# linjonathan/tropical_cyclone_risk

Measured on AMD Instinct MI355X. Metric: storm-steps/sec (100k-storm ensemble), higher is better.
Workload: dtype f64

## Files before the change

### include/tcrisk_hip.h

```cpp
#ifndef TCRISK_HIP_H
#define TCRISK_HIP_H

#include <stddef.h>
#include <stdint.h>

#ifdef __cplusplus
extern "C" {
#endif

#define TCR_ABI_VERSION 7
#define TCR_NW 4
#define TCR_NCOV 10
#define TCR_MAX_SERIES 32
#define TCR_N_BASINS 7

#define TCR_STATUS_GATED (-1)
#define TCR_STATUS_FINISHED 0
#define TCR_STATUS_EVENT 1
#define TCR_STATUS_STEP_FAIL (-2)
#define TCR_STATUS_STEP_OVERFLOW (-3)

#define TCR_FLAG_IS_TC 1
#define TCR_FLAG_ACCEPTED 2

// ... 49 lines not shown
    int32_t *nfev;
    int32_t *n_accept, *n_reject;
    int32_t *pad_state;
    int32_t tc_rows_only;
} tcr_tracks;

typedef struct {
    float *lon, *lat, *v, *m, *vmax;
    float *envw;
    int32_t *n_valid, *status, *flags, *nfev, *n_accept, *n_reject;
    int32_t *pad_state;
    int32_t tc_rows_only;
} tcr_tracks_f32;

int tcr_abi_version(void);
int tcr_ctx_create(int device, tcr_ctx **out);
int tcr_ctx_destroy(tcr_ctx *ctx);
const char *tcr_last_error(const tcr_ctx *ctx);

int tcr_params_set(tcr_ctx *ctx, const tcr_params *p);

int tcr_static_upload(tcr_ctx *ctx, const tcr_grid *hg, const double *land, const double *bathy);
int tcr_static_upload2(tcr_ctx *ctx, const tcr_grid *land_grid, const double *land,
                       const tcr_grid *bathy_grid, const double *bathy);
int tcr_static_store(tcr_ctx *ctx, int32_t pref);
int tcr_static_info(tcr_ctx *ctx, int32_t *mode, int64_t *bytes);
int tcr_fields_upload(tcr_ctx *ctx, int slot,
                      const tcr_grid *wg, const double *const mean[TCR_NW], const double *const cov[TCR_NCOV],
                      const tcr_grid *tg, const double *vpot, const double *chi,
                      const double *mld, const double *strat);
int tcr_rh_upload(tcr_ctx *ctx, int slot, const tcr_grid *rg, const double *rh_mid);
int tcr_slot_upload(tcr_ctx *ctx, int slot,
                    const tcr_grid *wg, const double *const mean[TCR_NW], const double *const cov[TCR_NCOV],
                    const tcr_grid *tg, const double *vpot, const double *chi, const double *mld, const double *strat,
                    const tcr_grid *rg, const double *rh_mid);
int tcr_stage_timing(tcr_ctx *ctx, double ms[5], int32_t reset);
int tcr_masks_upload(tcr_ctx *ctx, const tcr_grid *mg, const uint8_t *run_mask,
                     const uint8_t *const basin_masks[TCR_N_BASINS]);

int tcr_integrate_host(tcr_ctx *ctx, const tcr_storms *in, const tcr_tracks *out);
int tcr_integrate_dev(tcr_ctx *ctx, const tcr_storms *in_dev, const tcr_tracks *out_dev, void *stream);

int tcr_schedule_set(tcr_ctx *ctx, int32_t storms_per_lane);

typedef struct {
    int32_t waves;
    int32_t park;
    int32_t park_final;
    int32_t table_segments;
    int32_t prune;
    int32_t emit_grid_cap;
    int32_t copy_threads;
    int32_t table_factors;
} tcr_tune;
int tcr_tune_set(tcr_ctx *ctx, const tcr_tune *t);
int tcr_tune_get(tcr_ctx *ctx, tcr_tune *t);

int tcr_integrate_f32_dev(tcr_ctx *ctx, const tcr_storms *in_dev, const tcr_tracks_f32 *out_dev, void *stream);
int tcr_integrate_f32_host(tcr_ctx *ctx, const tcr_storms *in, const tcr_tracks_f32 *out);

typedef struct {
    int64_t n;
    double *lon0, *lat0, *v0, *m0, *h_bl;
    int32_t *slot;
    double *phases;
    int32_t *basin_idx;
    int32_t *seed_flags;
} tcr_seeds;
int tcr_seed_dev(tcr_ctx *ctx, uint64_t experiment_seed, int32_t year, int64_t cand0,
                 const tcr_seeds *out_dev, void *stream);
int tcr_seed_host(tcr_ctx *ctx, uint64_t experiment_seed, int32_t year, int64_t cand0,
                  const tcr_seeds *out_host);

int tcr_compact_dev(tcr_ctx *ctx, int64_t n, const int32_t *flags_dev, int32_t mask, int64_t max_out,
                    int32_t *idx_dev, int64_t *count_dev, void *stream);
int tcr_cell_order_dev(tcr_ctx *ctx, const tcr_seeds *cand_dev, int32_t *idx_dev, int64_t n, const int64_t *count_dev,
                       double cell_deg, void *stream);
int tcr_gather_seeds_dev(tcr_ctx *ctx, const tcr_seeds *src_dev, const int32_t *idx_dev, int64_t n_out,
                         const int64_t *count_dev, const tcr_seeds *dst_dev, uint64_t experiment_seed,
                         int32_t year, int64_t cand0, void *stream);
#define TCR_N_STATS 10
int tcr_stats_dev(tcr_ctx *ctx, int64_t n, const int64_t *n_dev, const tcr_tracks *tracks_dev, uint64_t *out_dev,
                  int32_t n_out, void *stream);
int tcr_pack_tracks_dev(tcr_ctx *ctx, const tcr_tracks *src_dev, const int32_t *idx_dev,
                        const int64_t *count_dev, int64_t cap, double *packed_dev, int64_t row_stride, void *stream);
int tcr_pack_tracks_f32_dev(tcr_ctx *ctx, const tcr_tracks_f32 *src_dev, const int32_t *idx_dev,
                            const int64_t *count_dev, int64_t cap, double *packed_dev, int64_t row_stride, void *stream);
int tcr_pack_tracks_meta_dev(tcr_ctx *ctx, const tcr_tracks *src_dev, int32_t f32, const int32_t *idx_dev,
                             const int64_t *count_dev, int64_t cap, double *packed_dev, int64_t row_stride,
                             const int32_t *cand_idx_dev, const int32_t *slot_dev, const int32_t *basin_idx_dev,
                             int64_t cand0, void *stream);
int tcr_seed_hist_dev(tcr_ctx *ctx, const tcr_seeds *cand_dev, int64_t cand0, const double *cutoff_dev,
                      int64_t *out_dev, void *stream);

typedef struct {
    int64_t n_cand;
    int64_t n_storms;
    tcr_seeds cand;
    tcr_seeds storms;
    int32_t *cand_idx;
    int64_t *n_passed;
    double cell_deg;
    int32_t exact_count;
    int32_t f32;
    tcr_tracks tracks;
    uint64_t *stats;
// ... 190 lines not shown
```

### tropical_cyclone_risk_amd/_lib.py

```python
import ctypes as C
import os

PKG_DIR = os.path.dirname(os.path.abspath(__file__))
LIB_PATH = os.path.join(PKG_DIR, 'libtcrisk_hip.so')

TCR_ABI_VERSION = 7
TCR_NW, TCR_NCOV, TCR_MAX_SERIES, TCR_N_BASINS = 4, 10, 32, 7
STATUS_GATED, STATUS_FINISHED, STATUS_EVENT, STATUS_STEP_FAIL, STATUS_STEP_OVERFLOW = -1, 0, 1, -2, -3
FLAG_IS_TC, FLAG_ACCEPTED = 1, 2
RAIN_TOTAL, RAIN_PEAK_RATE = 0, 1
SELECT_LDS_KEYS, SELECT_MAX_RANKS = 8192, 64
TAIL_MAX_K = 2048
STAGES = ('start', 'seed', 'select', 'order', 'gather', 'fourier', 'integrate', 'screen', 'select_tc', 'dense', 'emit', 'flags', 'stats', 'pack')
STATIC_MODES = ('f64', 'f64_split', 'pack16', 'u8_f32', 'pack64')
N_STATS = 10

DP = C.POINTER(C.c_double)
IP = C.POINTER(C.c_int32)
U8P = C.POINTER(C.c_uint8)

EXPORTS = ('tcr_abi_version', 'tcr_ctx_create', 'tcr_ctx_destroy', 'tcr_last_error',
           'tcr_params_set', 'tcr_static_upload', 'tcr_fields_upload', 'tcr_rh_upload', 'tcr_masks_upload',
           'tcr_integrate_host', 'tcr_integrate_dev', 'tcr_seed_dev', 'tcr_seed_host',
           'tcr_probe_rhs_host', 'tcr_fourier_table_host', 'tcr_timing_enable',
# ... 19 lines not shown
    _fields_ = [('nlon', C.c_int32), ('nlat', C.c_int32), ('lon', DP), ('lat', DP)]


class Params(C.Structure):
    _fields_ = [('Ck', C.c_double), ('epsilon', C.c_double), ('kappa', C.c_double),
                ('u_beta', C.c_double), ('v_beta', C.c_double), ('T_Fs', C.c_double),
                ('y_alpha', C.c_double * 2), ('m_alpha', C.c_double * 2),
                ('alpha_max', C.c_double * 2), ('alpha_min', C.c_double * 2),
                ('steering_coefs', C.c_double * 2),
                ('dt_out', C.c_double), ('total_time', C.c_double),
                ('rtol', C.c_double), ('atol', C.c_double), ('max_step', C.c_double),
                ('v_thresh', C.c_double), ('v_2d_thresh', C.c_double), ('vmax_thresh', C.c_double),
                ('v_dissipate', C.c_double), ('earth_R', C.c_double), ('box', C.c_double * 4),
                ('fs_amp', C.c_double), ('fs_wgt', C.c_double * TCR_MAX_SERIES),
                ('n_series', C.c_int32), ('n_steps', C.c_int32),
                ('coupled_track', C.c_int32), ('max_rk_steps', C.c_int32),
                ('seed_v_init', C.c_double), ('pi_gate', C.c_double), ('lat_vort_fac', C.c_double),
                ('lat_vort_power', C.c_double * TCR_N_BASINS),
                ('atm_bl_depth', C.c_double * TCR_N_BASINS),
                ('minit_a', C.c_double), ('minit_b', C.c_double),
                ('minit_c', C.c_double), ('minit_d', C.c_double)]


class Storms(C.Structure):
    _fields_ = [('n', C.c_int64), ('lon0', C.c_void_p), ('lat0', C.c_void_p), ('v0', C.c_void_p),
                ('m0', C.c_void_p), ('h_bl', C.c_void_p), ('slot', C.c_void_p), ('phases', C.c_void_p),
                ('n_dev', C.c_void_p)]


class Tracks(C.Structure):
    _fields_ = [('lon', C.c_void_p), ('lat', C.c_void_p), ('v', C.c_void_p), ('m', C.c_void_p),
                ('vmax', C.c_void_p), ('envw', C.c_void_p), ('n_valid', C.c_void_p),
                ('status', C.c_void_p), ('flags', C.c_void_p), ('nfev', C.c_void_p),
                ('n_accept', C.c_void_p), ('n_reject', C.c_void_p), ('pad_state', C.c_void_p),
                ('tc_rows_only', C.c_int32)]


class Seeds(C.Structure):
    _fields_ = [('n', C.c_int64), ('lon0', C.c_void_p), ('lat0', C.c_void_p), ('v0', C.c_void_p),
                ('m0', C.c_void_p), ('h_bl', C.c_void_p), ('slot', C.c_void_p),
                ('phases', C.c_void_p), ('basin_idx', C.c_void_p), ('seed_flags', C.c_void_p)]


class Round(C.Structure):
    _fields_ = [('n_cand', C.c_int64), ('n_storms', C.c_int64), ('cand', Seeds), ('storms', Seeds),
                ('cand_idx', C.c_void_p), ('n_passed', C.c_void_p), ('cell_deg', C.c_double),
                ('exact_count', C.c_int32), ('f32', C.c_int32), ('tracks', Tracks),
                ('stats', C.c_void_p), ('acc_idx', C.c_void_p), ('n_accepted', C.c_void_p),
                ('packed', C.c_void_p), ('pack_cap', C.c_int64), ('pack_stride', C.c_int64), ('seed_hist', C.c_void_p),
                ('n_expected', C.c_int64)]


class Tune(C.Structure):
    _fields_ = [(k, C.c_int32) for k in ('waves', 'park', 'park_final', 'table_segments', 'prune', 'emit_grid_cap', 'copy_threads', 'table_factors')]


class HazardTracks(C.Structure):
    _fields_ = [('n_trk', C.c_int64), ('n_t', C.c_int64), ('row_stride', C.c_int64), ('lon', C.c_void_p), ('lat', C.c_void_p),
                ('vmax', C.c_void_p), ('n_group', C.c_int32), ('group_off', C.POINTER(C.c_int64))]


class LandGrid(C.Structure):
    _fields_ = [('nlon', C.c_int64), ('nlat', C.c_int64), ('lon', C.c_void_p), ('lat', C.c_void_p), ('land', C.c_void_p)]


class ClimGrid(C.Structure):
    _fields_ = [('lon0', C.c_double), ('dlon', C.c_double), ('lat0', C.c_double), ('dlat', C.c_double), ('nlon', C.c_int64),
                ('nlat', C.c_int64)]


class ClimOut(C.Structure):
    _fields_ = [(k, C.c_void_p) for k in ('track', 'exceed', 'genesis', 'lmi', 'pdi', 'genesis_k', 'lmi_v', 'lmi_k', 'pdi_storm')]


class WindTracks(C.Structure):
    _fields_ = [('n_trk', C.c_int64), ('n_t', C.c_int64), ('row_stride', C.c_int64)] + \
        [(k, C.c_void_p) for k in ('lon', 'lat', 'v', 'u250', 'v250', 'u850', 'v850', 'rmax_km')] + \
        [('n_group', C.c_int32), ('group_off', C.POINTER(C.c_int64))]


class WindParams(C.Structure):
    _fields_ = [('dt_s', C.c_double), ('ck_cd', C.c_double), ('r_out_km', C.c_double), ('rmax_const_km', C.c_double),
                ('substeps', C.c_int32)]


class LossParams(C.Structure):
    _fields_ = [('v_thresh', C.c_double), ('v_half', C.c_double)]


class RainParams(C.Structure):
    _fields_ = [('dt_s', C.c_double), ('r_out_km', C.c_double), ('v_lo_kt', C.c_double), ('v_hi_kt', C.c_double),
                ('a', C.c_double * 4), ('b', C.c_double * 4), ('substeps', C.c_int32), ('stat', C.c_int32)]


class TcrError(RuntimeError):
    pass


_lib = None


def _pin_hip_runtime():
    import importlib.util
    import sys
    if 'torch' in sys.modules:
        return
    try:
# ... 145 lines not shown
```

### tropical_cyclone_risk_amd/csrc/tcr_abi.hip

```cpp
#include <hip/hip_runtime.h>

#include <cstdlib>

#include "tcr_kernels.hip"
#include "tcr_seed.hip"
#include "tcr_compact.hip"
#include "tcr_prep.hip"
#include "tcr_thermo.hip"
#ifdef TCR_EXPERIMENTS
#include "tcr_experiments.h"
#endif

#include "tcr_host.h"
#include "tcr_ctx.h"
#include "tcr_stage.hip"
#include "tcr_integrate.hip"
#include "tcr_preprocess.hip"
#include "tcr_round.hip"

namespace {

long env_long(const char *name, long dflt)
{
    const char *e = getenv(name);
    return e ? atol(e) : dflt;
}
tcr_tune tune_from_env()
{
    tcr_tune t;
    t.waves = (int32_t)env_long("TCR_WAVES", -1);
    t.park = (int32_t)std::min<long>(env_long("TCR_PARK", -1), 63);
    t.park_final = (int32_t)env_long("TCR_PARK_FINAL", -1);
    t.table_segments = (int32_t)env_long("TCR_TABLE_SEGMENTS", -1);
    t.prune = (int32_t)env_long("TCR_PRUNE", -1);
    t.emit_grid_cap = (int32_t)env_long("TCR_EMIT_GRID_CAP", -1);
    t.copy_threads = (int32_t)env_long("TCR_COPY_THREADS", -1);
    t.table_factors = (int32_t)env_long("TCR_TABLE_FACTORS", -1);
    return t;
}

}

extern "C" {

int tcr_abi_version(void) { return TCR_ABI_VERSION; }

const char *tcr_last_error(const tcr_ctx *ctx) { return ctx ? ctx->err.c_str() : g_create_error.c_str(); }

int tcr_ctx_create(int device, tcr_ctx **out)
{
    if (!out) return fail(nullptr, "tcr_ctx_create: out is NULL");
    *out = nullptr;
    int count = 0;
    hipError_t e = hipGetDeviceCount(&count);
    if (e != hipSuccess || count <= 0)
        return fail(nullptr, "no HIP device available (%s); this library has no CPU fallback",
                    e != hipSuccess ? hipGetErrorString(e) : "device count is 0");
    if (device < 0 || device >= count) return fail(nullptr, "tcr_ctx_create: device index out of range");
    tcr_ctx *ctx = new tcr_ctx();
    ctx->device = device;
    ctx->tune = tune_from_env();
    if (hipSetDevice(device) != hipSuccess || hipStreamCreate(&ctx->stream) != hipSuccess) {
        delete ctx;
        return fail(nullptr, "tcr_ctx_create: hipSetDevice/hipStreamCreate failed");
    }
    hipDeviceProp_t prop;
    if (hipGetDeviceProperties(&prop, device) == hipSuccess && prop.multiProcessorCount > 0) {
        ctx->cu_count = prop.multiProcessorCount;
        if (prop.sharedMemPerBlock < kCellScanLds) {
            delete ctx;
            return fail(nullptr, "tcr_ctx_create: this library is built for gfx950 (160 KB of LDS per CU); the device offers less than k_cell_scan's 67 KB per workgroup");
        }
    }
    if (ctx->ws.d_queue.alloc_bytes(kQueueWords * sizeof(unsigned long long)) != hipSuccess ||
        ctx->ws.d_tc_count.alloc_bytes(64) != hipSuccess || ctx->rd.d_round_key.alloc_bytes(64) != hipSuccess) {
        delete ctx;
        return fail(nullptr, "tcr_ctx_create: hipMalloc failed");
    }
    *out = ctx;
    return 0;
}

int tcr_ctx_destroy(tcr_ctx *ctx)
{
    if (!ctx) return 0;
    (void)hipSetDevice(ctx->device);
    (void)hipStreamSynchronize(ctx->stream);
    delete ctx;
    return 0;
}
// ... 71 lines not shown
```

### tropical_cyclone_risk_amd/csrc/tcr_integrate.hip

```cpp
#pragma once
#include <cmath>

#include "tcr_stage.hip"

namespace {

unsigned integrate_waves(const tcr_ctx *ctx, int64_t n, int wps)
{
    (void)wps;
    const int64_t simds = (int64_t)ctx->cu_count * 4;
    int64_t waves = (n + kWave - 1) / kWave;
    if (ctx->tune.waves > 0) return (unsigned)(ctx->tune.waves < waves ? ctx->tune.waves : waves);
    if (waves > simds) waves = (n >= simds * kWave * 4) ? 2 * simds : simds;
    else if (ctx->storms_per_lane > 1) {
        const int64_t w = (n + (int64_t)kWave * ctx->storms_per_lane - 1) / ((int64_t)kWave * ctx->storms_per_lane);
        waves = std::max<int64_t>(std::min<int64_t>(waves, 16), w);
    }
    return (unsigned)(waves < 1 ? 1 : waves);
}

int park_threshold(const tcr_ctx *ctx, unsigned waves, int wps)
{
    if (ctx->tune.park >= 0) return ctx->tune.park > 63 ? 63 : ctx->tune.park;
    (void)wps;
// ... 120 lines not shown
            int list_stride = 1;
            if (part == kFsRest) {
                list = reinterpret_cast<const int64_t *>(park) + 13;
                list_stride = kParkRec;
            } else if (!fused) {
                if (W.d_pf.grow(ctx, (size_t)tiles * kFsMfmaKSteps * 32) < 0) return -1;
                hipLaunchKernelGGL(k_phase_factors_frag, dim3((unsigned)std::min<int64_t>(tiles, 8192)), dim3(256), 0, st, P, n, n_dev, phases,
                                   reinterpret_cast<double *>(W.d_pf.p), nullptr, nullptr, z);
            }
            const double *p = fused ? phases : reinterpret_cast<const double *>(W.d_pf.p);
            const int groups = part == kFsAll ? kFsMfmaColGroups : 1;
            int64_t want = (int64_t)ctx->cu_count * kFsMfmaWgsPerCu * (4 / kFsMfmaWaves) / groups;
#ifdef TCR_EXPERIMENTS
            want = tcr_exp::fs_workgroups(want, groups);
#endif
            const unsigned wgs = (unsigned)std::min<int64_t>(tiles, std::max<int64_t>(1, want));
            const dim3 grid(wgs, groups), block(64 * kFsMfmaWaves);
            const BatchReset none{};
            with_flags(part == kFsRest, fused, [&](auto REST, auto FUSED) {
                constexpr bool rest = decltype(REST)::value, fu = decltype(FUSED)::value;
                hipLaunchKernelGGL((k_fourier_mfma<R, rest, fu>), grid, block, 0, st, P, n, n_dev, W.fs_period, W.d_sc_table.p, p, fs,
                                   rest ? 1 : 0, list, list_stride, park_count, (fu && !rest) ? z : none);
            });
        } else {
            hipLaunchKernelGGL(k_phase_factors, dim3((unsigned)((nf + 255) / 256)), dim3(256), 0, st, P, n, n_dev, phases, W.d_pf.p);
            hipLaunchKernelGGL(k_fourier_periodic<R>, dim3((unsigned)n), dim3(kFsThreads), lds, st, P, n, n_dev,
                               W.fs_period, W.d_sc_table.p, W.d_pf.p, fs);
        }
    } else {
        const int64_t total = n * (int64_t)P.n_steps;
        hipLaunchKernelGGL(k_fourier_direct<R>, dim3((unsigned)((total + 255) / 256)), dim3(256), 0, st, P, n, n_dev, phases, fs);
    }
    HIPCHK(ctx, hipGetLastError());
    return 0;
}

template <typename R>
int integrate_impl(tcr_ctx *ctx, const tcr_storms *in, const TracksT<R> out, void *stream_, uint64_t *stats = nullptr,
                   const int64_t *stats_n_dev = nullptr, int64_t n_expected = 0)
{
    hipStream_t st = enter(ctx, stream_);
    if (!st) return -1;
    IntegrateWs &W = ctx->ws;
    const int64_t n = in->n;
    if (n < 0) return fail(ctx, "tcr_integrate: negative n");
    if (n == 0) return 0;
    const tcr_params &P = ctx->prm;
    const size_t ns = (size_t)P.n_steps;
    constexpr size_t REC = (size_t)step_rec_doubles<R>();
    if (W.d_fs.grow(ctx, ((size_t)n * ns * 4 * sizeof(R) + 7) / 8) < 0) return -1;
    const int max_rk = P.max_rk_steps > 0 ? P.max_rk_steps : 64;
    if (W.d_srec.grow(ctx, (size_t)n * max_rk * REC) < 0) return -1;
    if (max_rk > 65535) return fail(ctx, "tcr_params.max_rk_steps must be <= 65535");
    if (W.d_sidx.grow(ctx, ((size_t)n * ns * sizeof(uint16_t) + 7) / 8 * 4) < 0) return -1;
    R *fs = reinterpret_cast<R *>(W.d_fs.p);
    EvalKT<R> EK{};
    bool affine = false;
    if (eval_k_ready<R>(ctx, EK, &affine, st)) return -1;

    hipEvent_t *ev = nullptr;
    if (ctx->tr.timing && !ctx->capturing && timing_events(ctx, &ev)) return -1;
    if (ev) HIPCHK(ctx, hipEventRecord(ev[0], st));
    const int wps = std::is_same<R, double>::value ? TCR_INT_WPS : TCR_INT_WPS_F32;
    unsigned waves = integrate_waves(ctx, (n_expected > 0 && n_expected < n) ? n_expected : n, wps);
    const int thr = park_threshold(ctx, waves, wps);
    const unsigned final_waves = park_final_waves(ctx);
    const bool segmented = kFsMfmaColGroups == 2 && thr > 0 && waves > final_waves && kMaxPasses > 1 && fourier_on_matrix_cores(ctx) &&
                           (int)P.n_steps > kFsSegSamples + 16 && ctx->tune.table_segments != 0;
    int prune_sample = -1;
    if (out.tc_rows_only && ctx->tune.prune != 0) {
        const double t2d = 2 * 86400.0, step_out = P.total_time / (double)(P.n_steps - 1);
        const int j = (int)floor(t2d / step_out);
        if (j >= 1 && j < P.n_steps - 1 && ts_host(P, j) == t2d) prune_sample = j;
    }
    const bool in_flight = prune_sample >= 0;
    if (!in_flight && W.d_vrec.grow(ctx, (size_t)n * max_rk * kVRec) < 0) return -1;
    if (out.tc_rows_only && W.d_tc_idx.grow(ctx, (size_t)n) < 0) return -1;
    unsigned long long *tc_count = reinterpret_cast<unsigned long long *>(W.d_tc_count.p);
    {
        BatchReset z{};
        z.queue = W.d_queue.p; z.queue_words = (int)kQueueWords;
        if (in_flight) { z.flags = out.flags; z.n_flags = n; }
        if (out.tc_rows_only) z.tc_count = tc_count;
        if (launch_fourier<R>(ctx, n, in->n_dev, in->phases, fs, st, segmented ? kFsFirst : kFsAll, nullptr, nullptr, &z)) return -1;
    }
    STAGE(TCR_STAGE_FOURIER);
    if (ev) HIPCHK(ctx, hipEventRecord(ev[1], st));
    {
        KArgsT<R> a{};
        a.P = P; a.D = dev_fields(ctx); a.K = EK; a.n = n; a.n_dev = in->n_dev;
        a.lon0 = in->lon0; a.lat0 = in->lat0; a.v0 = in->v0; a.m0 = in->m0; a.h_bl = in->h_bl;
        a.slot = in->slot; a.phases = in->phases; a.fs = fs; a.srec = W.d_srec.p; a.vrec = in_flight ? nullptr : W.d_vrec.p; a.max_rk_steps = max_rk;
        a.n_valid = out.n_valid; a.status = out.status; a.nfev = out.nfev;
        a.n_accept = out.n_accept; a.n_reject = out.n_reject;
        a.queue = W.d_queue.p;
        a.prune_sample = prune_sample;
        if (in_flight) {
            a.tc_list = W.d_tc_idx.p; a.tc_count = tc_count;
        }
        const size_t park_items = segmented ? (size_t)n : (size_t)waves * kWave;
        if (thr > 0 && W.d_park[0].grow(ctx, park_items * kParkRec) < 0) return -1;
        if (thr > 0 && W.d_park[1].grow(ctx, park_items * kParkRec) < 0) return -1;
        const bool probe = std::is_same<R, double>::value && W.d_probe;
        if (probe) { a.probe = W.d_probe; a.probe_cap = W.probe_cap; }
        bool seg_events = false;
        for (int pass = 0; pass < kMaxPasses; ++pass) {
            const bool last = thr <= 0 || waves <= final_waves || pass == kMaxPasses - 1;
            a.pass = pass;
            a.fill_pct = pass_fill_pct();
            a.threshold = last ? 0 : thr;
            a.park_in = W.d_park[(pass + 1) & 1].p;
            a.park_out = W.d_park[pass & 1].p;
            a.t_limit = (segmented && pass == 0) ? ts_host(P, kFsSegSamples - 2) : 1e300;
            launch_integrate(a, affine, probe, ctx->sg.static_mode, waves, st);
            if (last) break;
            if (segmented && pass == 0) {
                if (ev) HIPCHK(ctx, hipEventRecord(ev[4], st));
                if (launch_fourier<R>(ctx, n, in->n_dev, in->phases, fs, st, kFsRest, W.d_park[0].p, W.d_queue.p + kMaxPasses)) return -1;
                if (ev) HIPCHK(ctx, hipEventRecord(ev[5], st));
                seg_events = true;
                continue;
            }
            waves = (unsigned)(((size_t)waves * (size_t)(thr - 1) + kWave - 1) / kWave);
        }
        if (ev && !seg_events) { HIPCHK(ctx, hipEventRecord(ev[4], st)); HIPCHK(ctx, hipEventRecord(ev[5], st)); }
    }
    STAGE(TCR_STAGE_INTEGRATE);
    if (W.d_steps) HIPCHK(ctx, hipMemcpyAsync(W.d_steps, W.d_srec.p, sizeof(double) * (size_t)n * max_rk * REC, hipMemcpyDeviceToDevice, st));
    if (ev) HIPCHK(ctx, hipEventRecord(ev[2], st));
    {
        EArgsT<R> a{};
        a.P = P; a.D = dev_fields(ctx); a.n = n; a.n_dev = in->n_dev; a.max_rk_steps = max_rk; a.srec = W.d_srec.p; a.vrec = in_flight ? nullptr : W.d_vrec.p; a.fs = fs;
        a.slot = in->slot; a.n_valid = out.n_valid; a.status = out.status; a.n_accept = out.n_accept;
        a.lon = out.lon; a.lat = out.lat; a.v = out.v; a.m = out.m; a.vmax = out.vmax;
        a.envw = out.envw; a.flags = out.flags; a.pad_state = out.pad_state;
        a.K = EK;
        const unsigned chunks = (unsigned)((ns + kPostThreads - 1) / kPostThreads);
        if (out.tc_rows_only) {
            if (!in_flight) {
                a.tc_list = W.d_tc_idx.p; a.tc_count = tc_count;
                hipLaunchKernelGGL(k_screen<R>, dim3((unsigned)((n + kScreenStorms - 1) / kScreenStorms)), dim3(kScreenThreads), 0, st, a);
            }
            STAGE(TCR_STAGE_SCREEN);
            STAGE(TCR_STAGE_SELECT_TC);
            a.list = W.d_tc_idx.p; a.count = W.d_tc_count.p;
        }
        int64_t cap = kEmitGridCap;
        if (ctx->tune.emit_grid_cap > 0) cap = ctx->tune.emit_grid_cap;
        const unsigned gx = (out.tc_rows_only && n > 2 * cap) ? (unsigned)cap : (unsigned)n;
        hipLaunchKernelGGL(k_dense<R>, dim3(gx), dim3(kWave), 0, st, a, W.d_sidx.p);
        STAGE(TCR_STAGE_DENSE);
        const unsigned ex = gx;
        auto emit = [&](unsigned rows, bool overflow) {
            with_flags(affine, overflow, [&](auto A, auto OV) {
                hipLaunchKernelGGL((k_emit<R, decltype(A)::value, decltype(OV)::value>), dim3(rows, chunks), dim3(kPostThreads), 0, st, a, W.d_sidx.p);
            });
        };
        emit(ex, false);
        if ((int64_t)ex < n) {
            a.item_base = ex;
            emit((unsigned)std::min<int64_t>(n - ex, 256), true);
            a.item_base = 0;
        }
        STAGE(TCR_STAGE_EMIT);
        hipLaunchKernelGGL(k_flags<R>, dim3((unsigned)((n + 255) / 256)), dim3(256), 0, st, P, n, out.n_valid,
                           out.status, out.v, out.flags, out.pad_state, out.tc_rows_only ? 1 : 0, a.n_dev, out.nfev,
                           reinterpret_cast<unsigned long long *>(stats), stats_n_dev);
        STAGE(TCR_STAGE_FLAGS);
    }
    if (ev) HIPCHK(ctx, hipEventRecord(ev[3], st));
    HIPCHK(ctx, hipGetLastError());
    return 0;
}

int storms_upload(tcr_ctx *ctx, DevBuf &B, const tcr_storms *in, tcr_storms *d, const char *who, bool need_m0 = true)
{
    const size_t n = (size_t)in->n;
    for (size_t i = 0; i < n; ++i)
        if (!slot_staged(ctx, in->slot[i])) return fail(ctx, "%s: storm references a slot that is not staged", who);
    *d = tcr_storms{};
    d->n = in->n;
    d->lon0 = B.put(in->lon0, n); d->lat0 = B.put(in->lat0, n); d->v0 = B.put(in->v0, n);
    d->m0 = (need_m0 || in->m0) ? B.put(in->m0, n) : nullptr;
    d->h_bl = B.put(in->h_bl, n); d->slot = B.put(in->slot, n);
    d->phases = B.put(in->phases, n * 4 * (size_t)ctx->prm.n_series);
    d->n_dev = nullptr;
    if (!d->lon0 || !d->lat0 || !d->v0 || ((need_m0 || in->m0) && !d->m0) || !d->h_bl || !d->slot || !d->phases)
        return fail(ctx, "%s: device allocation / upload failed", who);
    return 0;
}

template <typename R, typename T>
int integrate_host_impl(tcr_ctx *ctx, const tcr_storms *in, const T *out)
{
    if (ready(ctx, false)) return -1;
    if (!in || !out) return fail(ctx, "tcr_integrate_host: NULL argument");
    if (!enter(ctx)) return -1;
    const size_t n = (size_t)in->n, ns = (size_t)ctx->prm.n_steps;
    if (n == 0) return 0;
    DevBuf B;
    tcr_storms di{};
    if (storms_upload(ctx, B, in, &di, "tcr_integrate_host")) return -1;
    TracksT<R> dout{};
    dout.lon = B.get<R>(n * ns); dout.lat = B.get<R>(n * ns); dout.v = B.get<R>(n * ns);
    dout.m = B.get<R>(n * ns); dout.vmax = B.get<R>(n * ns); dout.envw = B.get<R>(n * ns * 4);
    dout.n_valid = B.get<int32_t>(n); dout.status = B.get<int32_t>(n); dout.flags = B.get<int32_t>(n);
    dout.nfev = B.get<int32_t>(n); dout.n_accept = B.get<int32_t>(n); dout.n_reject = B.get<int32_t>(n);
    if (!dout.lon || !dout.lat || !dout.v || !dout.m || !dout.vmax || !dout.envw || !dout.n_valid || !dout.status ||
// ... 302 lines not shown
```

### tropical_cyclone_risk_amd/csrc/tcr_kernels.hip

```cpp
#include "tcr_device.h"

namespace tcr {

template <typename R>
struct KArgsT {
    tcr_params P;
    DevFields D;
    EvalKT<R> K;
    int64_t n;
    const int64_t *n_dev;
    const double *lon0, *lat0, *v0, *m0, *h_bl;
    const int32_t *slot;
    const double *phases;
    R *fs;
    double *srec;
    int32_t *n_valid, *status, *nfev, *n_accept, *n_reject;
    unsigned long long *queue;
    int max_rk_steps;
    int pass;
    int threshold;
    int fill_pct;
    const double *park_in;
    double *park_out;
    double t_limit;
// ... 794 lines not shown
};
using EArgs = EArgsT<double>;
static_assert(sizeof(EvalKT<double>) % 8 == 0 && sizeof(EvalKT<float>) % 8 == 0, "EvalK is copied to LDS in eight-byte words");
constexpr int kBitAny15 = 1 << 8, kBitVmax = 1 << 9;
constexpr int kBitListed = 1 << 10;
#ifndef TCR_POST_THREADS
#define TCR_POST_THREADS 128
#endif
constexpr int kPostThreads = TCR_POST_THREADS;
#ifndef TCR_EMIT_GRID_CAP
#define TCR_EMIT_GRID_CAP 8192
#endif
constexpr int64_t kEmitGridCap = TCR_EMIT_GRID_CAP;
constexpr int kEmitSlotCache = 32;
#ifndef TCR_EMIT_WPS
#define TCR_EMIT_WPS 3
#endif
#ifndef TCR_SHADOW_WPS
#define TCR_SHADOW_WPS 6
#endif

template <typename R>
__device__ __forceinline__ const R *rec_body(const double *rec) { return reinterpret_cast<const R *>(rec + kStepHdr); }

template <typename R>
__global__ __launch_bounds__(kWave) void k_dense(EArgsT<R> a, uint16_t *__restrict__ sidx)
{
    const tcr_params &P = a.P;
    const int64_t n_items = a.list ? *a.count : a.n;
    const int64_t n_exist = a.list ? n_items : n_eff(a.n, a.n_dev);
    for (int64_t item = blockIdx.x; item < n_items; item += gridDim.x) {
        if (item >= n_exist) {
            if (threadIdx.x == 0) a.flags[item] = 0;
            continue;
        }
        const int64_t sid = a.list ? (int64_t)a.list[item] : item;
        const int ns = P.n_steps;
        const int n = a.n_valid[sid];
        int nst = a.n_accept[sid];
        nst = nst < a.max_rk_steps ? nst : a.max_rk_steps;
        if (threadIdx.x == 0) a.flags[sid] = a.list ? kBitListed : 0;
        constexpr int REC = step_rec_doubles<R>();
        typedef typename VecT<R, 4>::type V4;
        const int c = threadIdx.x & 3;
        for (int j0 = 0; j0 < nst; j0 += kWave / 4) {
            const int j = j0 + (threadIdx.x >> 2);
            const bool on = j < nst;
            double *rj = const_cast<double *>(a.srec) + (sid * (int64_t)a.max_rk_steps + (on ? j : 0)) * REC;
            R *body = reinterpret_cast<R *>(rj + kStepHdr);
            R kq[7];
            for (int q = 0; q < 7; ++q) kq[q] = body[4 + q * 4 + c];
            const double t_old = rj[0], t_new = rj[2];
            R Q[4];
            for (int k = 0; k < 4; ++k) {
                R acc = R(0.0);
                for (int q = 0; q < 7; ++q) acc += kq[q] * R(RK_P[q][k]);
                Q[k] = acc;
            }
            if (on) {
                V4 qv; qv[0] = Q[0]; qv[1] = Q[1]; qv[2] = Q[2]; qv[3] = Q[3];
                *reinterpret_cast<V4 *>(body + 4 + c * 4) = qv;
                if (c == 0) {
                    const int i_lo = (j == 0) ? 0 : samples_upto(P, t_old);
                    int i_hi = samples_upto(P, t_new);
                    i_hi = i_hi < n ? i_hi : n;
                    for (int i = i_lo; i < i_hi; ++i) sidx[(size_t)sid * ns + i] = (uint16_t)j;
                }
            }
        }
    }
}

template <typename R>
__device__ __forceinline__ R haversine_same_lat_km(const tcr_params &P, R lon1, R lon2, R lat)
{
    const R d = R(kPi / 180.0);
    lon1 *= d; lon2 *= d; lat *= d;
    const R sb = sin((lon2 - lon1) / R(2)), c = cos(lat);
    const R aa = R(0.0) + c * c * (sb * sb);
    return R(P.earth_R / 1000.) * (R(2) * asin(sqrt(aa)));
}

template <typename R>
__device__ __forceinline__ R haversine_same_lon_km(const tcr_params &P, R lat1, R lat2)
{
    const R d = R(kPi / 180.0);
    lat1 *= d; lat2 *= d;
    const R sa = sin((lat2 - lat1) / R(2));
    const R aa = sa * sa;
    return R(P.earth_R / 1000.) * (R(2) * asin(sqrt(aa)));
}

template <typename R>
__device__ __forceinline__ R vmax_at(const tcr_params &P, R lon, R lat, R v, R us, R vs, R lom, R lam, R lop, R lap)
{
    const R dlon = R(0.5) * (sign_of(lop - lom) * haversine_same_lat_km<R>(P, lop, lom, lat));
    const R dlat = R(0.5) * (sign_of(lap - lam) * haversine_same_lon_km<R>(P, lap, lam));
    const R ut = dlon * R(1000.) / (R)P.dt_out, vt = dlat * R(1000.) / (R)P.dt_out;
    const R G = fmin(R(1.), R(0.8) + R(0.35) * (R(1.) + tanh((lat - R(35.)) / R(10.))));
    const R Ui = G * ut + R(0.1) * us * v / R(15.);
    const R Vi = G * vt + R(0.1) * vs * v / R(15.);
    const R mag = sqrt(Ui * Ui + Vi * Vi);
    const R fac = np_min((v * R(0.50)) / mag, R(1.0));
    const R msin = (mag == R(0.0)) ? R(0.0) : Ui / mag;
    const R mcos = (mag == R(0.0)) ? R(1.0) : Vi / mag;
    const R ug = v * msin + Ui * fac;
    const R vg = v * mcos + Vi * fac;
    return sqrt(ug * ug + vg * vg);
}

template <typename R, int NC>
__device__ __forceinline__ void dense_at(const double *__restrict__ srec_storm, int step, double te, R (&ye)[NC])
{
    typedef typename VecT<R, 4>::type V4;
    const double *rec = srec_storm + (size_t)step * step_rec_doubles<R>();
    const double2 h0 = *reinterpret_cast<const double2 *>(rec);
    const V4 *body = reinterpret_cast<const V4 *>(rec + kStepHdr);
    const R hh = (R)h0.y;
    const R x = (R)((te - h0.x) / h0.y);
    const R p1 = x, p2 = p1 * x, p3 = p2 * x, p4 = p3 * x;
    const V4 y0 = body[0];
#pragma unroll
    for (int c = 0; c < NC; ++c) {
        const V4 q = body[1 + c];
        R acc = R(0.0);
        acc += q[0] * p1; acc += q[1] * p2; acc += q[2] * p3; acc += q[3] * p4;
        ye[c] = hh * acc + y0[c];
    }
}

template <typename R, bool AFFINE, bool LIST>
__global__ __launch_bounds__(kPostThreads, TCR_SHADOW_WPS) void k_emit(EArgsT<R> a, const uint16_t *__restrict__ sidx)
{
    __shared__ EvalKT<R> K_lds;
    __shared__ const R *s_wind[kEmitSlotCache];
    const tcr_params &P = a.P;
    const int64_t n_items = a.list ? *a.count : n_eff(a.n, a.n_dev);
    if ((int64_t)blockIdx.x + (LIST ? a.item_base : 0) >= n_items) return;
    const int ns = P.n_steps;
    const int i = blockIdx.y * kPostThreads + threadIdx.x;
    const R nan = (R)__longlong_as_double(0x7ff8000000000000LL);
    for (unsigned w = threadIdx.x; w < sizeof(EvalKT<R>) / 8; w += kPostThreads)
        reinterpret_cast<uint64_t *>(&K_lds)[w] = reinterpret_cast<const uint64_t *>(&a.K)[w];
    if (threadIdx.x < kEmitSlotCache && (int)threadIdx.x < a.D.n_slots) s_wind[threadIdx.x] = slot_wind<R>(a.D.slots[threadIdx.x]);
    __syncthreads();
    int64_t item = blockIdx.x + (LIST ? a.item_base : 0);
#pragma unroll 1
    do {
        int koff = 0;
        asm volatile("" : "+s"(koff));
        const EvalKT<R> &K = *reinterpret_cast<const EvalKT<R> *>(reinterpret_cast<const char *>(&K_lds) + koff);
        const int64_t sid = a.list ? (int64_t)a.list[item] : item;
        const int n = a.n_valid[sid];
        const int slot_id = a.slot[sid];
        const uint16_t *sidx_storm = sidx + (size_t)sid * ns;
        const int my_step = (i < ns) ? sidx_storm[i] : 0;
        const size_t o = (size_t)sid * ns + i;
        typedef typename VecT<R, 4>::type V4;
        const bool valid = i < n;
        const double *srec_storm = a.srec + sid * (int64_t)a.max_rk_steps * step_rec_doubles<R>();
        R ye[4] = {0, 0, 0, 0}, w[4] = {0, 0, 0, 0};
        if (valid) {
            const double te = ts_at(P, i);
            dense_at<R, 4>(srec_storm, my_step, te, ye);
            const R *wind = (slot_id < kEmitSlotCache) ? s_wind[slot_id] : slot_wind<R>(a.D.slots[slot_id]);
            env_winds<R, AFFINE>(K, wind, a.fs + sid * ns * 4, ye[0], ye[1], te, w);
            a.lon[o] = ye[0]; a.lat[o] = ye[1]; a.v[o] = ye[2]; a.m[o] = ye[3];
            V4 wv; wv[0] = w[0]; wv[1] = w[1]; wv[2] = w[2]; wv[3] = w[3];
            *reinterpret_cast<V4 *>(a.envw + o * 4) = wv;
        }
        const int lane = threadIdx.x & 63;
        R lom = __shfl_up(ye[0], 1), lam = __shfl_up(ye[1], 1);
        R lop = __shfl_down(ye[0], 1), lap = __shfl_down(ye[1], 1);
        if (valid && n > 1) {
            if (lane == 0 && i > 0) {
                R q[2];
                dense_at<R, 2>(srec_storm, sidx_storm[i - 1], ts_at(P, i - 1), q);
                lom = q[0]; lam = q[1];
            }
            if (lane == 63 && i < n - 1) {
                R q[2];
                dense_at<R, 2>(srec_storm, sidx_storm[i + 1], ts_at(P, i + 1), q);
                lop = q[0]; lap = q[1];
            }
            const R lop_in = lop, lap_in = lap, lom_in = lom, lam_in = lam;
            if (i == 0) { lom = R(2) * ye[0] - lop_in; lam = R(2) * ye[1] - lap_in; }
            if (i == n - 1) { lop = R(2) * ye[0] - lom_in; lap = R(2) * ye[1] - lam_in; }
            const R vm = vmax_at<R>(P, ye[0], ye[1], ye[2], w[0] - w[2], w[1] - w[3], lom, lam, lop, lap);
            a.vmax[o] = vm;
            const bool hit_v = ye[2] >= (R)P.v_thresh, hit_vm = vm >= (R)P.vmax_thresh;
            const int bits = (__ballot(hit_v) ? kBitAny15 : 0) | (__ballot(hit_vm) ? kBitVmax : 0);
            if (bits && lane == (__ffsll((long long)__ballot(true)) - 1)) atomicOr(a.flags + sid, bits);
        } else if (valid) {
            a.vmax[o] = nan;
            if (ye[2] >= (R)P.v_thresh) atomicOr(a.flags + sid, kBitAny15);
        } else {
            int pad_to = a.pad_state ? a.pad_state[sid] : ns;
            pad_to = (pad_to < 0 || pad_to > ns) ? ns : pad_to;
            if (i < pad_to) {
                a.lon[o] = nan; a.lat[o] = nan; a.v[o] = nan; a.m[o] = nan; a.vmax[o] = nan;
                V4 nv; nv[0] = nan; nv[1] = nan; nv[2] = nan; nv[3] = nan;
                *reinterpret_cast<V4 *>(a.envw + o * 4) = nv;
            }
        }
    } while (LIST && (item += gridDim.x) < n_items);
}

constexpr int kScreenThreads = 256;
constexpr int kScreenGroup = 16;
constexpr int kScreenStorms = kScreenThreads / kScreenGroup;

template <typename R>
__global__ __launch_bounds__(kScreenThreads, TCR_SHADOW_WPS) void k_screen(EArgsT<R> a)
{
    __shared__ R cap[kScreenStorms][3];
    const tcr_params &P = a.P;
    const int g = threadIdx.x / kScreenGroup, l = threadIdx.x % kScreenGroup;
    const int64_t sid = (int64_t)blockIdx.x * kScreenStorms + g;
    const bool on = sid < a.n;
    const bool exists = sid < n_eff(a.n, a.n_dev);
    const int ns = P.n_steps;
    int n = 0, nst = 0, st = TCR_STATUS_GATED;
    if (exists) {
        n = a.n_valid[sid]; nst = a.n_accept[sid]; st = a.status[sid];
        nst = nst < a.max_rk_steps ? nst : a.max_rk_steps;
    }
    const double step_out = P.total_time / (double)(ns - 1);
    const double t2d = 2 * 86400.0;
    const bool clamp2d = n > 0 && t2d >= ts_at(P, n - 1);
    const int j2d = clamp2d ? n - 1 : (int)floor(t2d / step_out);
    bool any15 = false;
    const double *vrec_storm = a.vrec + sid * (int64_t)a.max_rk_steps * kVRec;
    typedef StepVT<R> StepV;
    auto load_step = [&](int j) {
        const double2 *rj = reinterpret_cast<const double2 *>(vrec_storm + (size_t)j * kVRec);
        const double2 r0 = rj[0], r1 = rj[1], r2 = rj[2], r3 = rj[3], r4 = rj[4], r5 = rj[5];
        StepV s;
        s.t_old = r0.x; s.h64 = r0.y;
        const double t_new = r1.x;
        s.hh = (R)s.h64; s.y0 = (R)r1.y;
        const R kq[7] = {(R)r2.x, (R)r2.y, (R)r3.x, (R)r3.y, (R)r4.x, (R)r4.y, (R)r5.x};
        dense_v_row<R>(kq, s.Q);
        s.i_lo = (j == 0) ? 0 : samples_upto(P, s.t_old);
        s.i_hi = samples_upto(P, t_new);
        s.i_hi = s.i_hi < n ? s.i_hi : n;
        return s;
    };
    auto v_at = [&](const StepV &s, int i) -> R { return dense_v_at<R>(P, s, i); };
    auto caps = [&](const StepV &s) {
        if (s.i_lo <= j2d && j2d < s.i_hi) cap[g][0] = v_at(s, j2d);
        if (s.i_lo <= j2d + 1 && j2d + 1 < s.i_hi) cap[g][1] = v_at(s, j2d + 1);
        if (s.i_lo <= n - 1 && n - 1 < s.i_hi) cap[g][2] = v_at(s, n - 1);
    };
    const bool has0 = l < nst && n > 0;
    StepV s0{};
    if (has0) { s0 = load_step(l); caps(s0); }
    for (int j = l + kScreenGroup; j < nst && n > 0; j += kScreenGroup) caps(load_step(j));
    __syncthreads();
// ... 240 lines not shown
```

Measured before the change: 11.25 billion.

## Fold dense-output step conversion into emit kernel, dropping the separate dense pass

Makes fusion the default: the emit kernel now builds the sample-to-step ownership map in LDS, computes the dense-output polynomial coefficients for the RK steps covering its chunk, and evaluates the track samples and edge neighbours from shared memory. This removes the separate k_dense launch and the global sidx buffer along with its write and read traffic. The old two-pass path stays available through a TCR_DENSE_PASS tune knob. The cost is more shared memory, extra block syncs per group of steps, and recomputing coefficients for steps shared by neighbouring chunks.

Result: no change. 11.33 billion, median of 6 (+0.7%).

```diff
diff --git a/include/tcrisk_hip.h b/include/tcrisk_hip.h
--- a/include/tcrisk_hip.h
+++ b/include/tcrisk_hip.h
@@ -125,6 +125,7 @@
     int32_t emit_grid_cap;
     int32_t copy_threads;
     int32_t table_factors;
+    int32_t dense_pass;
 } tcr_tune;
 int tcr_tune_set(tcr_ctx *ctx, const tcr_tune *t);
 int tcr_tune_get(tcr_ctx *ctx, tcr_tune *t);
diff --git a/tropical_cyclone_risk_amd/_lib.py b/tropical_cyclone_risk_amd/_lib.py
--- a/tropical_cyclone_risk_amd/_lib.py
+++ b/tropical_cyclone_risk_amd/_lib.py
@@ -95,7 +95,7 @@
 
 
 class Tune(C.Structure):
-    _fields_ = [(k, C.c_int32) for k in ('waves', 'park', 'park_final', 'table_segments', 'prune', 'emit_grid_cap', 'copy_threads', 'table_factors')]
+    _fields_ = [(k, C.c_int32) for k in ('waves', 'park', 'park_final', 'table_segments', 'prune', 'emit_grid_cap', 'copy_threads', 'table_factors', 'dense_pass')]
 
 
 class HazardTracks(C.Structure):
diff --git a/tropical_cyclone_risk_amd/csrc/tcr_abi.hip b/tropical_cyclone_risk_amd/csrc/tcr_abi.hip
--- a/tropical_cyclone_risk_amd/csrc/tcr_abi.hip
+++ b/tropical_cyclone_risk_amd/csrc/tcr_abi.hip
@@ -36,6 +36,7 @@
     t.emit_grid_cap = (int32_t)env_long("TCR_EMIT_GRID_CAP", -1);
     t.copy_threads = (int32_t)env_long("TCR_COPY_THREADS", -1);
     t.table_factors = (int32_t)env_long("TCR_TABLE_FACTORS", -1);
+    t.dense_pass = (int32_t)env_long("TCR_DENSE_PASS", -1);
     return t;
 }
 
diff --git a/tropical_cyclone_risk_amd/csrc/tcr_integrate.hip b/tropical_cyclone_risk_amd/csrc/tcr_integrate.hip
--- a/tropical_cyclone_risk_amd/csrc/tcr_integrate.hip
+++ b/tropical_cyclone_risk_amd/csrc/tcr_integrate.hip
@@ -196,7 +196,8 @@
     const int max_rk = P.max_rk_steps > 0 ? P.max_rk_steps : 64;
     if (W.d_srec.grow(ctx, (size_t)n * max_rk * REC) < 0) return -1;
     if (max_rk > 65535) return fail(ctx, "tcr_params.max_rk_steps must be <= 65535");
-    if (W.d_sidx.grow(ctx, ((size_t)n * ns * sizeof(uint16_t) + 7) / 8 * 4) < 0) return -1;
+    const bool fold = ctx->tune.dense_pass <= 0;
+    if (!fold && W.d_sidx.grow(ctx, ((size_t)n * ns * sizeof(uint16_t) + 7) / 8 * 4) < 0) return -1;
     R *fs = reinterpret_cast<R *>(W.d_fs.p);
     EvalKT<R> EK{};
     bool affine = false;
@@ -224,7 +225,7 @@
     {
         BatchReset z{};
         z.queue = W.d_queue.p; z.queue_words = (int)kQueueWords;
-        if (in_flight) { z.flags = out.flags; z.n_flags = n; }
+        if (in_flight || fold) { z.flags = out.flags; z.n_flags = n; }
         if (out.tc_rows_only) z.tc_count = tc_count;
         if (launch_fourier<R>(ctx, n, in->n_dev, in->phases, fs, st, segmented ? kFsFirst : kFsAll, nullptr, nullptr, &z)) return -1;
     }
@@ -292,12 +293,14 @@
         int64_t cap = kEmitGridCap;
         if (ctx->tune.emit_grid_cap > 0) cap = ctx->tune.emit_grid_cap;
         const unsigned gx = (out.tc_rows_only && n > 2 * cap) ? (unsigned)cap : (unsigned)n;
-        hipLaunchKernelGGL(k_dense<R>, dim3(gx), dim3(kWave), 0, st, a, W.d_sidx.p);
+        if (!fold) hipLaunchKernelGGL(k_dense<R>, dim3(gx), dim3(kWave), 0, st, a, W.d_sidx.p);
         STAGE(TCR_STAGE_DENSE);
         const unsigned ex = gx;
         auto emit = [&](unsigned rows, bool overflow) {
             with_flags(affine, overflow, [&](auto A, auto OV) {
-                hipLaunchKernelGGL((k_emit<R, decltype(A)::value, decltype(OV)::value>), dim3(rows, chunks), dim3(kPostThreads), 0, st, a, W.d_sidx.p);
+                constexpr bool AF = decltype(A)::value, ov = decltype(OV)::value;
+                if (fold) hipLaunchKernelGGL((k_emit<R, AF, ov>), dim3(rows, chunks), dim3(kPostThreads), 0, st, a);
+                else hipLaunchKernelGGL((k_emit_sidx<R, AF, ov>), dim3(rows, chunks), dim3(kPostThreads), 0, st, a, W.d_sidx.p);
             });
         };
         emit(ex, false);
diff --git a/tropical_cyclone_risk_amd/csrc/tcr_kernels.hip b/tropical_cyclone_risk_amd/csrc/tcr_kernels.hip
--- a/tropical_cyclone_risk_amd/csrc/tcr_kernels.hip
+++ b/tropical_cyclone_risk_amd/csrc/tcr_kernels.hip
@@ -870,11 +870,7 @@
             for (int q = 0; q < 7; ++q) kq[q] = body[4 + q * 4 + c];
             const double t_old = rj[0], t_new = rj[2];
             R Q[4];
-            for (int k = 0; k < 4; ++k) {
-                R acc = R(0.0);
-                for (int q = 0; q < 7; ++q) acc += kq[q] * R(RK_P[q][k]);
-                Q[k] = acc;
-            }
+            dense_v_row<R>(kq, Q);
             if (on) {
                 V4 qv; qv[0] = Q[0]; qv[1] = Q[1]; qv[2] = Q[2]; qv[3] = Q[3];
                 *reinterpret_cast<V4 *>(body + 4 + c * 4) = qv;
@@ -947,11 +943,38 @@
     }
 }
 
-template <typename R, bool AFFINE, bool LIST>
-__global__ __launch_bounds__(kPostThreads, TCR_SHADOW_WPS) void k_emit(EArgsT<R> a, const uint16_t *__restrict__ sidx)
+template <typename R, int NC>
+__device__ __forceinline__ void dense_at(const double2 h0, const R *__restrict__ body_lds, double te, R (&ye)[NC])
+{
+    typedef typename VecT<R, 4>::type V4;
+    const V4 *body = reinterpret_cast<const V4 *>(body_lds);
+    const R hh = (R)h0.y;
+    const R x = (R)((te - h0.x) / h0.y);
+    const R p1 = x, p2 = p1 * x, p3 = p2 * x, p4 = p3 * x;
+    const V4 y0 = body[0];
+#pragma unroll
+    for (int c = 0; c < NC; ++c) {
+        const V4 q = body[1 + c];
+        R acc = R(0.0);
+        acc += q[0] * p1; acc += q[1] * p2; acc += q[2] * p3; acc += q[3] * p4;
+        ye[c] = hh * acc + y0[c];
+    }
+}
+
+constexpr int kFoldSteps = 16;
+constexpr int kFoldBody = 20;
+static_assert(kFoldSteps * 4 <= kPostThreads, "k_emit's fold: a lane per (step, component)");
+
+template <typename R, bool AFFINE, bool LIST, bool FOLD>
+__device__ __forceinline__ void emit_body(const EArgsT<R> &a, const uint16_t *__restrict__ sidx)
 {
     __shared__ EvalKT<R> K_lds;
     __shared__ const R *s_wind[kEmitSlotCache];
+    __shared__ double2 s_hdr[FOLD ? kFoldSteps : 1];
+    __shared__ __attribute__((aligned(32))) R s_body[FOLD ? kFoldSteps * kFoldBody : 4];
+    __shared__ uint16_t s_own[FOLD ? kPostThreads + 2 : 2];
+    __shared__ R s_v[FOLD ? kPostThreads : 1];
+    __shared__ R s_edge[kPostThreads / 64][4];
     const tcr_params &P = a.P;
     const int64_t n_items = a.list ? *a.count : n_eff(a.n, a.n_dev);
     if ((int64_t)blockIdx.x + (LIST ? a.item_base : 0) >= n_items) return;
@@ -971,34 +994,97 @@
         const int64_t sid = a.list ? (int64_t)a.list[item] : item;
         const int n = a.n_valid[sid];
         const int slot_id = a.slot[sid];
-        const uint16_t *sidx_storm = sidx + (size_t)sid * ns;
-        const int my_step = (i < ns) ? sidx_storm[i] : 0;
+        const uint16_t *sidx_storm = FOLD ? nullptr : sidx + (size_t)sid * ns;
+        const int my_step = (!FOLD && i < ns) ? sidx_storm[i] : 0;
         const size_t o = (size_t)sid * ns + i;
         typedef typename VecT<R, 4>::type V4;
         const bool valid = i < n;
         const double *srec_storm = a.srec + sid * (int64_t)a.max_rk_steps * step_rec_doubles<R>();
         R ye[4] = {0, 0, 0, 0}, w[4] = {0, 0, 0, 0};
+        const bool edge_m = valid && n > 1 && (threadIdx.x & 63) == 0 && i > 0, edge_p = valid && n > 1 && (threadIdx.x & 63) == 63 && i < n - 1;
+        if (FOLD) {
+            if (a.list && blockIdx.y == 0 && threadIdx.x == 0) atomicOr(a.flags + sid, kBitListed);
+            const int i0 = blockIdx.y * kPostThreads;
+            if (i0 < n) {
+                constexpr int REC = step_rec_doubles<R>();
+                int nst = a.n_accept[sid];
+                nst = nst < a.max_rk_steps ? nst : a.max_rk_steps;
+                const int w_lo = i0 > 0 ? i0 - 1 : 0, w_hi = (i0 + kPostThreads + 1 < n) ? i0 + kPostThreads + 1 : n;
+                for (int j = threadIdx.x; j < nst; j += kPostThreads) {
+                    const double *rj = srec_storm + (size_t)j * REC;
+                    const double t_old = rj[0], t_new = rj[2];
+                    int i_lo = (j == 0) ? 0 : samples_upto(P, t_old);
+                    int i_hi = samples_upto(P, t_new);
+                    i_hi = i_hi < w_hi ? i_hi : w_hi;
+                    i_lo = i_lo > w_lo ? i_lo : w_lo;
+                    for (int k = i_lo; k < i_hi; ++k) s_own[k - (i0 - 1)] = (uint16_t)j;
+                }
+                __syncthreads();
+                const int j_top = nst > 0 ? nst - 1 : 0;
+                auto own = [&](int k) { const int j = s_own[k - (i0 - 1)]; return j < j_top ? j : j_top; };
+                const int j_first = own(w_lo), j_last = own(w_hi - 1);
+                const int my_j = valid ? own(i) : 0, jm = edge_m ? own(i - 1) : 0, jp = edge_p ? own(i + 1) : 0;
+                const double te = ts_at(P, i);
+#pragma unroll 1
+                for (int jb = j_first; jb <= j_last; jb += kFoldSteps) {
+                    if (jb != j_first) __syncthreads();
+                    const int s = threadIdx.x >> 2, c = threadIdx.x & 3, j = jb + s;
+                    if (s < kFoldSteps && j <= j_last) {
+                        const double *rj = srec_storm + (size_t)j * REC;
+                        const R *body = rec_body<R>(rj);
+                        R kq[7];
+                        for (int q = 0; q < 7; ++q) kq[q] = body[4 + q * 4 + c];
+                        const R y_old = body[c];
+                        if (c == 0) s_hdr[s] = *reinterpret_cast<const double2 *>(rj);
+                        R Q[4];
+                        dense_v_row<R>(kq, Q);
+                        V4 qv; qv[0] = Q[0]; qv[1] = Q[1]; qv[2] = Q[2]; qv[3] = Q[3];
+                        *reinterpret_cast<V4 *>(&s_body[s * kFoldBody + 4 + c * 4]) = qv;
+                        s_body[s * kFoldBody + c] = y_old;
+                    }
+                    __syncthreads();
+                    const unsigned span = (unsigned)(j_last - jb < kFoldSteps - 1 ? j_last - jb : kFoldSteps - 1);
+                    if (valid && (unsigned)(my_j - jb) <= span) dense_at<R, 4>(s_hdr[my_j - jb], &s_body[(my_j - jb) * kFoldBody], te, ye);
+                    if (edge_m && (unsigned)(jm - jb) <= span) {
+                        R q[2];
+                        dense_at<R, 2>(s_hdr[jm - jb], &s_body[(jm - jb) * kFoldBody], ts_at(P, i - 1), q);
+                        s_edge[threadIdx.x >> 6][0] = q[0]; s_edge[threadIdx.x >> 6][1] = q[1];
+                    }
+                    if (edge_p && (unsigned)(jp - jb) <= span) {
+                        R q[2];
+                        dense_at<R, 2>(s_hdr[jp - jb], &s_body[(jp - jb) * kFoldBody], ts_at(P, i + 1), q);
+                        s_edge[threadIdx.x >> 6][2] = q[0]; s_edge[threadIdx.x >> 6][3] = q[1];
+                    }
+                }
+            }
+        }
         if (valid) {
             const double te = ts_at(P, i);
-            dense_at<R, 4>(srec_storm, my_step, te, ye);
+            if (!FOLD) dense_at<R, 4>(srec_storm, my_step, te, ye);
+            if (FOLD) { a.m[o] = ye[3]; s_v[threadIdx.x] = ye[2]; asm volatile("" ::: "memory"); }
             const R *wind = (slot_id < kEmitSlotCache) ? s_wind[slot_id] : slot_wind<R>(a.D.slots[slot_id]);
             env_winds<R, AFFINE>(K, wind, a.fs + sid * ns * 4, ye[0], ye[1], te, w);
-            a.lon[o] = ye[0]; a.lat[o] = ye[1]; a.v[o] = ye[2]; a.m[o] = ye[3];
+            if (FOLD) { asm volatile("" ::: "memory"); ye[2] = s_v[threadIdx.x]; }
+            a.lon[o] = ye[0]; a.lat[o] = ye[1]; a.v[o] = ye[2];
+            if (!FOLD) a.m[o] = ye[3];
             V4 wv; wv[0] = w[0]; wv[1] = w[1]; wv[2] = w[2]; wv[3] = w[3];
             *reinterpret_cast<V4 *>(a.envw + o * 4) = wv;
         }
-        const int lane = threadIdx.x & 63;
+        const int lane = FOLD ? (int)__builtin_amdgcn_mbcnt_hi(~0u, __builtin_amdgcn_mbcnt_lo(~0u, 0u)) : (int)(threadIdx.x & 63);
         R lom = __shfl_up(ye[0], 1), lam = __shfl_up(ye[1], 1);
         R lop = __shfl_down(ye[0], 1), lap = __shfl_down(ye[1], 1);
         if (valid && n > 1) {
-            if (lane == 0 && i > 0) {
+            if (FOLD) asm volatile("" ::: "memory");
+            if (edge_m) {
                 R q[2];
-                dense_at<R, 2>(srec_storm, sidx_storm[i - 1], ts_at(P, i - 1), q);
+                if (FOLD) { q[0] = s_edge[threadIdx.x >> 6][0]; q[1] = s_edge[threadIdx.x >> 6][1]; }
+                else dense_at<R, 2>(srec_storm, sidx_storm[i - 1], ts_at(P, i - 1), q);
                 lom = q[0]; lam = q[1];
             }
-            if (lane == 63 && i < n - 1) {
+            if (edge_p) {
                 R q[2];
-                dense_at<R, 2>(srec_storm, sidx_storm[i + 1], ts_at(P, i + 1), q);
+                if (FOLD) { q[0] = s_edge[threadIdx.x >> 6][2]; q[1] = s_edge[threadIdx.x >> 6][3]; }
+                else dense_at<R, 2>(srec_storm, sidx_storm[i + 1], ts_at(P, i + 1), q);
                 lop = q[0]; lap = q[1];
             }
             const R lop_in = lop, lap_in = lap, lom_in = lom, lam_in = lam;
@@ -1022,6 +1108,18 @@
             }
         }
     } while (LIST && (item += gridDim.x) < n_items);
+}
+
+template <typename R, bool AFFINE, bool LIST>
+__global__ __launch_bounds__(kPostThreads, TCR_SHADOW_WPS) void k_emit(EArgsT<R> a)
+{
+    emit_body<R, AFFINE, LIST, true>(a, nullptr);
+}
+
+template <typename R, bool AFFINE, bool LIST>
+__global__ __launch_bounds__(kPostThreads, TCR_SHADOW_WPS) void k_emit_sidx(EArgsT<R> a, const uint16_t *__restrict__ sidx)
+{
+    emit_body<R, AFFINE, LIST, false>(a, sidx);
 }
 
 constexpr int kScreenThreads = 256;
```
